# xiaguan/yalm

Measured on AMD Instinct MI355X. Metric: decode tok/s Mistral-7B fp16 @1 GPU; % of HBM bytes/token roofline, higher is better.
Workload: dtype f16; 1 GPU; mistral-7b fp16 batch-1 greedy decode, 1163 tokens, kv_len 19..1181; model=mistral-7b, global_batch=1, seq_len=1181, parallelism=single

## Files before the change

include/yalm_hip.h:

```cpp
#ifndef YALM_HIP_H
#define YALM_HIP_H

#include <stddef.h>
#include <stdint.h>

#ifdef __cplusplus
extern "C" {
#endif

#define YALM_OK 0
#define YALM_ERR_HIP 1
#define YALM_ERR_ARG 2
#define YALM_ERR_UNSUPPORTED 3

enum { YALM_F32 = 0, YALM_F16 = 1, YALM_BF16 = 2, YALM_F8E5M2 = 3 };
enum { YALM_Q4 = 16 };
enum { YALM_GELU = 0, YALM_SILU = 1 };
enum { YALM_HYDRATE_KV_CACHE = 0, YALM_OUTPUT_LOGITS = 1 };

typedef struct yalm_stream_s *yalm_stream;
typedef struct yalm_decoder_s *yalm_decoder;

typedef struct yalm_config {
	int dim, hidden_dim, head_dim, n_layers, n_heads, n_kv_heads, vocab_size, max_seq_len;
// ... 53 lines not shown
int yalm_set_x(yalm_decoder d, const float *host);
int yalm_get_logits(yalm_decoder d, float *host);
int yalm_time_kernel(yalm_decoder d, int kernel_id, int iters, float *avg_ms);
int yalm_stream_envelope(size_t bytes, int iters, float *avg_ms);
int yalm_set_gemv_config(yalm_decoder d, int kind, int threads, int unroll, int gpw);
int yalm_graph_kernels(yalm_decoder d, int mode, int *kernels, int *nodes);
const char *yalm_kernel_name(yalm_decoder d, int kernel_id);
int yalm_decoder_attn_wo(yalm_decoder d);
#define YALM_LAUNCH_EAGER 1
#define YALM_LAUNCH_SYNC 2
#define YALM_LAUNCH_SEPARATE_ATTN_WO 4
int yalm_decoder_set_launch(yalm_decoder d, int flags);
int yalm_attn_wo_plan(const yalm_config *config, int slots, int *splits, int *grid);
int yalm_attn_wo_trace(yalm_decoder d, unsigned long long *host, size_t count, int *workgroups,
                       int *attention_workgroups);

typedef struct yalm_rope_scaling {
	int type;
	float factor, low_freq_factor, high_freq_factor;
	int original_max_position;
} yalm_rope_scaling;
int yalm_decoder_set_rope_scaling(yalm_decoder d, const yalm_rope_scaling *s);
int yalm_decoder_get_inv_freq(yalm_decoder d, float *host);
int yalm_decoder_set_qkv_bias(yalm_decoder d, const float *const *bq, const float *const *bk,
                              const float *const *bv);

typedef struct yalm_moe_config {
	int n_experts, n_experts_active;
} yalm_moe_config;
int yalm_decoder_create_moe(const yalm_config *config, const yalm_moe_config *moe, const yalm_model_weights *weights,
// ... 69 lines not shown
```

yalm_amd/csrc/attention.h:

```cpp
#pragma once

#include <float.h>

#include <type_traits>

#include "device_common.h"

#define ATTN_THREADS 256
#define ATTN_SPLITS 32
#define ATTN_MAX_SPLITS 64
#define ATTN_HEAD_MAX 4
#define ATTN_WAVES (ATTN_THREADS / YALM_WAVE)

template <int D>
constexpr int attn_chunk() {
	return 64;
}

template <int D>
constexpr int attn_nk() {
	return attn_chunk<D>() / (ATTN_WAVES * (64 / (D / 8))) > 0 ? attn_chunk<D>() / (ATTN_WAVES * (64 / (D / 8))) : 1;
}

template <int D>
struct KvRows {
	static constexpr int LPK = D / 8, KPW = 64 / LPK, RSTEP = (ATTN_THREADS / 64) * KPW;
	static constexpr int NK = attn_nk<D>();
	const char *kb, *vb;
	uint32_t rowb, msl;
	uint32_t voff[NK];
	__device__ __forceinline__ KvRows(const uint16_t *kc, const uint16_t *vc, int n_kv_heads, int max_seq_len, int g) {
		const int lane = threadIdx.x & 63;
		const int tl0 = (threadIdx.x >> 6) * KPW + lane / LPK, piece = lane % LPK;
		auto uni = [](const uint16_t *p) {
			const uint64_t a = (uint64_t)p;
			const uint32_t lo = __builtin_amdgcn_readfirstlane((uint32_t)a);
// ... 105 lines not shown
	case 12: return dpp<0x15C>(v);
	case 13: return dpp<0x15D>(v);
	case 14: return dpp<0x15E>(v);
	default: return dpp<0x15F>(v);
	}
}
template <int LPK, bool MAX>
__device__ __forceinline__ float attn_wave_red(float v) {
	auto op = [](float a, float b) { return MAX ? fmaxf(a, b) : a + b; };
	v = attn_fold_row<LPK, MAX>(v);
	if constexpr (LPK <= 16)
		v = op(v, xor16(v));
	return op(v, xor32(v));
}

template <int D, int GT, int GQ, bool GRAN>
__device__ __forceinline__ bool attn_core(int g, int hq0, int Gh, int c_first, int cstride, int ns, bool final_out,
                                          int s_part, const float4_t (&qv)[(GQ * D + 255) / 256],
                                          u32x4_t (&kA)[attn_nk<D>()], u32x4_t (&vA)[attn_nk<D>()],
                                          int kv_len, const uint16_t *kc, const uint16_t *vc, int n_heads,
                                          int n_kv_heads, int max_seq_len, int nsplit, unsigned long long *part,
                                          unsigned ptag, float *out, float *att_dbg, unsigned gtag,
                                          unsigned long long *ts, bool trace_on) {
	constexpr int CHUNK = attn_chunk<D>();
	c_first = __builtin_amdgcn_readfirstlane(c_first);
	cstride = __builtin_amdgcn_readfirstlane(cstride);
	ns = __builtin_amdgcn_readfirstlane(ns);
	kv_len = __builtin_amdgcn_readfirstlane(kv_len);
	constexpr int LPK = D / 8;
	static_assert(LPK >= 2 && LPK <= 32 && (LPK & (LPK - 1)) == 0, "head_dim 16 .. 256, a power of two");
	constexpr int KPW = 64 / LPK;
	constexpr int RSTEP = ATTN_WAVES * KPW;
	constexpr int NK = CHUNK / RSTEP > 0 ? CHUNK / RSTEP : 1;
	constexpr int QL = (GQ * D + 255) / 256;
// ... 16 lines not shown
	auto stamp = [&](int k) {
		if (ts) {
			tss[k] = __builtin_amdgcn_s_memrealtime();
			tss[8 + k] = __builtin_amdgcn_s_memtime();
		}
	};
	auto flush = [&]() {
		if (ts) {
#pragma unroll
			for (int k = 2; k < 8; ++k)
				if (k != 3)
					ts[k] = tss[k], ts[8 + k] = tss[8 + k];
		}
	};
	if (trace_on) {
		asm volatile("s_waitcnt vmcnt(0)" ::: "memory");
		__syncthreads();
		stamp(2);
	}
	const int gq = G * D;
#pragma unroll
	for (int j = 0; j < QL; ++j)
		if ((j * 64 + lane) * 4 < gq)
			*(float4_t *)&qs[wave][(j * 64 + lane) * 4] = qv[j];
	float qr[GT][8];
#pragma unroll
	for (int h = 0; h < GT; ++h) {
		const float *qp = &qs[wave][(hq0 + (h < Gh ? h : 0)) * D + piece * 8];
		const float4_t a = *(const float4_t *)qp;
		const float4_t b = *(const float4_t *)(qp + 4);
		qr[h][0] = a[0], qr[h][1] = a[1], qr[h][2] = a[2], qr[h][3] = a[3];
// ... 144 lines not shown
#pragma unroll
			for (int i = 0; i < NK; ++i) {
				float vf[8];
				WF16::unpack(valid[i] ? vw[i] : u32x4_t{0u, 0u, 0u, 0u}, vf);
#pragma unroll
				for (int h = 0; h < GT; ++h)
#pragma unroll
					for (int e = 0; e < 8; ++e)
						acc[h * 8 + e] = fmaf(sv[i][h], vf[e], acc[h * 8 + e]);
			}
		}
	};

	using T_ = std::true_type;
	using F_ = std::false_type;
	if (c_first + cstride >= ns) {
		chunk(T_{}, kA, vA, c_first * CHUNK);
	} else {
		u32x4_t kB[NK], vB[NK];
		load_kv((c_first + cstride) * CHUNK, kB, vB);
		chunk(T_{}, kA, vA, c_first * CHUNK);
		for (int c = c_first + cstride;; c += 2 * cstride) {
			load_kv((c + cstride) * CHUNK, kA, vA);
			chunk(F_{}, kB, vB, c * CHUNK);
			if (c + cstride >= ns)
				break;
			load_kv((c + 2 * cstride) * CHUNK, kB, vB);
			chunk(F_{}, kA, vA, (c + cstride) * CHUNK);
			if (c + 2 * cstride >= ns)
				break;
		}
// ... 77 lines not shown
			for (int w = 1; w < ATTN_WAVES; ++w)
				M = fmaxf(M, wml[w][h][0]);
			float L = 0.0f;
#pragma unroll
			for (int w = 0; w < ATTN_WAVES; ++w)
				L = fmaf(wml[w][h][1], expf(wml[w][h][0] - M), L);
			float *a = att_dbg + (size_t)(hb + h) * max_seq_len + t;
			*a = expf(ld_sc1(a) - M) / L;
		}
	}
	flush();
	return final_out;
}

template <int D, int GT, bool GRAN>
__device__ __forceinline__ bool attn_decode_body(int g, int u, int S, int head_max, const float *q,
                                                 const uint16_t *kc, const uint16_t *vc, const StepState *step,
                                                 int n_heads, int n_kv_heads, int max_seq_len, int nsplit,
                                                 unsigned long long *part, unsigned ptag, float *out, float *att_dbg,
                                                 unsigned gtag = 0, unsigned long long *ts = nullptr,
                                                 bool trace_on = false) {
	constexpr int CHUNK = attn_chunk<D>();
	constexpr int LPK = D / 8;
	constexpr int KPW = 64 / LPK;
	constexpr int RSTEP = ATTN_WAVES * KPW;
	constexpr int NK = CHUNK / RSTEP > 0 ? CHUNK / RSTEP : 1;
	constexpr int QL = (GT * D + 255) / 256;
	const int G = n_heads / n_kv_heads;
	const int lane = threadIdx.x & 63;
	const bool hu = u < G;
	const int s = hu ? 0 : u - G + 1;
	const int gq = G * D;
	float4_t qv[QL];
#pragma unroll
	for (int j = 0; j < QL; ++j)
		qv[j] = *(const float4_t *)(q + (size_t)g * gq + min((j * 64 + lane) * 4, gq - 4));
	u32x4_t kA[NK], vA[NK];
	const KvRows<D> rows(kc, vc, n_kv_heads, max_seq_len, g);
	rows.load(0, hu, kA, vA);
	const int kv_len = step->kv_len;
	const int ns = (kv_len + CHUNK - 1) / CHUNK;
	if (ns <= head_max) {
		if (!hu)
			return false;
		return attn_core<D, 1, GT, GRAN>(g, u, 1, 0, 1, ns, true, 0, qv, kA, vA, kv_len, kc, vc, n_heads, n_kv_heads,
		                                 max_seq_len, nsplit, part, ptag, out, att_dbg, gtag, ts, trace_on);
	}
	if (s * CHUNK >= kv_len)
		return false;
	if (!hu)
		rows.load(s * CHUNK, true, kA, vA);
	if (hu)
		return attn_core<D, 1, GT, GRAN>(g, u, 1, 0, S, ns, false, 0, qv, kA, vA, kv_len, kc, vc, n_heads, n_kv_heads,
		                                 max_seq_len, nsplit, part, ptag, out, att_dbg, gtag, ts, trace_on);
	return attn_core<D, GT, GT, GRAN>(g, 0, G, s, S, ns, false, s, qv, kA, vA, kv_len, kc, vc, n_heads, n_kv_heads,
	                                  max_seq_len, nsplit, part, ptag, out, att_dbg, gtag, ts, trace_on);
}

template <int D, bool GRAN>
__device__ __forceinline__ bool attn_merge_body(int g, int hq, int S, int head_max, const StepState *step, int n_heads,
                                                int n_kv_heads, int max_seq_len, int nsplit,
                                                const unsigned long long *part, unsigned ptag, unsigned *err,
                                                float *out, float *att_dbg, unsigned gtag = 0,
                                                unsigned long long *ts = nullptr) {
	constexpr int CHUNK = attn_chunk<D>();
	constexpr int SPW = ATTN_MAX_SPLITS / ATTN_WAVES;
	constexpr int E = D >= 64 ? D / 64 : 1;
	__shared__ float mml[ATTN_WAVES][2];
	__shared__ float mo[ATTN_WAVES][D];
	const int G = n_heads / n_kv_heads;
	const int h = g * G + hq;
// ... 85 lines not shown
	for (int d = tid; d < D; d += ATTN_THREADS)
		attn_out<GRAN>(out, (size_t)h * D + d, ((mo[0][d] + mo[1][d]) + (mo[2][d] + mo[3][d])) / L, gtag);
	if (att_dbg) {
		for (int t = tid; t < kv_len; t += ATTN_THREADS) {
			float *a = att_dbg + (size_t)h * max_seq_len + t;
			*a = expf(ld_sc1(a) - M) / L;
		}
	}
	return true;
}

template <int D, int GT>
__global__ __launch_bounds__(ATTN_THREADS) void attn_decode_kernel(
    const float *__restrict__ q, const uint16_t *__restrict__ kc, const uint16_t *__restrict__ vc,
    const StepState *__restrict__ step, int n_heads, int n_kv_heads, int max_seq_len, int nsplit, int S,
    int head_max, unsigned long long *__restrict__ part, int layer, int n_layers, unsigned *__restrict__ err,
    float *__restrict__ out, float *__restrict__ att_dbg) {
	const int b = blockIdx.x, units = n_kv_heads * (S + n_heads / n_kv_heads - 1);
	const unsigned ptag = attn_part_tag(step, layer, n_layers);
	if (b < units)
		attn_decode_body<D, GT, false>(b % n_kv_heads, b / n_kv_heads, S, head_max, q, kc, vc, step, n_heads,
		                               n_kv_heads, max_seq_len, nsplit, part, ptag, out, att_dbg);
	else
		attn_merge_body<D, false>((b - units) % n_kv_heads, (b - units) / n_kv_heads, S, head_max, step, n_heads,
		                          n_kv_heads, max_seq_len, nsplit, part, ptag, err, out, att_dbg);
}
```

yalm_amd/csrc/attn_wo.h:

```cpp
#pragma once

#include "attention.h"
#include "device_common.h"
#include "tp_exchange.h"

#define AWO_RPW 16
#define AWO_TIMEOUT 200000000ull
#define AWO_REPL_STRIDE 32
#define AWO_SHORT_KV 64
#define AWO_TRACE_N 16

struct AttnWoArgs {
	int n_heads, n_kv, max_seq_len, nsplit, S;
	int head_max;
	int q_dim, dim;
	unsigned long long *part;
	int layer, n_layers;
	const unsigned long long *gran;
	const char *wo;
	float *x;
	float *out;
	int add_base;
	TpX push;
	unsigned *err;
	unsigned long long *trace;
	int delay;
};

__device__ __forceinline__ void awo_ld8_sc1(u32x4_t (&v)[8], const void *const (&a)[8]) {
// ... 97 lines not shown
	unsigned long long t_start = 0, c_start = 0;
	if (tr) {
		t_start = __builtin_amdgcn_s_memrealtime();
		c_start = (unsigned long long)__builtin_amdgcn_s_getreg((31 << 11) | 4) |
		          ((unsigned long long)__builtin_amdgcn_s_getreg((31 << 11) | 20) << 32);
	}

	const unsigned epoch = step->epoch;
	if (b < munits) {
		const unsigned ptag = epoch * (unsigned)p.n_layers + (unsigned)p.layer;
		if (tr) {
			tr[2] = tr[10] = 0;
			for (int k = 4; k < 8; ++k)
				tr[k] = tr[8 + k] = 0;
		}
		const bool wrote =
		    b < units ? attn_decode_body<D, GT, true>(b % p.n_kv, b / p.n_kv, p.S, p.head_max, q, kc, vc, step,
		                                               p.n_heads, p.n_kv, p.max_seq_len, p.nsplit, p.part, ptag,
		                                               (float *)p.gran, nullptr, epoch, tr, p.trace != nullptr)
		              : attn_merge_body<D, true>((b - units) % p.n_kv, (b - units) / p.n_kv, p.S, p.head_max, step,
		                                         p.n_heads, p.n_kv, p.max_seq_len, p.nsplit, p.part, ptag, p.err,
		                                         (float *)p.gran, nullptr, epoch, tr);
		if (tr) {
			const unsigned long long t1 = __builtin_amdgcn_s_memrealtime(), c1 = __builtin_amdgcn_s_memtime();
			tr[0] = t_start, tr[8] = c_start;
			tr[1] = wrote ? t1 : 0, tr[9] = wrote ? c1 : 0;
			tr[3] = t1, tr[11] = c1;
		}
		return;
	}

	__shared__ float rowpart[AWO_RPW][ATTN_WAVES];
// ... 83 lines not shown
```

yalm_amd/csrc/decoder.h:

```cpp
#pragma once

#include <hip/hip_runtime.h>

#include <cstdlib>
#include <string>
#include <vector>

#include "../../include/yalm_hip.h"
#include "device_common.h"
#include "tp_exchange.h"

void set_err(const std::string &s);

#define HIPCHK(expr)                                                                                                   \
	do {                                                                                                               \
		hipError_t e_ = (expr);                                                                                        \
		if (e_ != hipSuccess) {                                                                                        \
			set_err(std::string(#expr) + " failed: " + hipGetErrorString(e_) + " (" + __FILE__ + ":" +                 \
			        std::to_string(__LINE__) + ")");                                                                   \
			return YALM_ERR_HIP;                                                                                       \
		}                                                                                                              \
	} while (0)

#define ARGCHK(cond, msg)                                                                                              \
// ... 103 lines not shown
	int ipc_S = 0;
	float *ipc_own = nullptr;
	float **ipc_bufs = nullptr;
	std::vector<void *> ipc_opened;
	TpX tpx{};
	bool tpx_gate = false;
	bool tpx_collect = false;
	bool attn_wo = false, attn_wo_ok = false;
	int awo_nb = 0;
	int awo_S = 0;
	int awo_slots = 0;
	unsigned long long *awo_trace = nullptr;
	int awo_delay = 0;
	int awo_delay_short = -1;
	long long awo_kv_hint = -1;
	unsigned long long *awo_gran = nullptr;
	unsigned *awo_err = nullptr;
	int moe_E = 0, moe_K = 0;
	StepState *rstep = nullptr;
	float *rx = nullptr, *rq = nullptr, *rxb2 = nullptr, *rhb = nullptr, *rlogits = nullptr;
	float *rlogits_pinned = nullptr;
	struct SpecState *spec = nullptr;
	int *spec_ctx = nullptr;
	int *spec_stream = nullptr;
	int spec_stream_cap = 0;
	yalm_rope_scaling rope_scaling{};
	std::vector<const float *> bq, bk, bv;
	std::vector<const void *> moegate;
	int *moe_sel = nullptr;
	float *moe_wts = nullptr;
// ... 5 lines not shown
```

yalm_amd/csrc/yalm_hip.hip:

```cpp
#include "../../include/yalm_hip.h"

#include <hip/hip_runtime.h>
#include <rccl/rccl.h>

#include <algorithm>
#include <cmath>
#include <cstddef>
#include <cstdio>
#include <cstdlib>
#include <cstring>
#include <string>
#include <vector>

#include "attention.h"
#include "attn_wo.h"
#include "decoder.h"
#include "device_common.h"
#include "gemv.h"
#include "gemv_rows.h"
#include "misc_kernels.h"
#include "moe.h"
#include "sampler.h"
#include "spec.h"

// ... 415 lines not shown
	ARGCHK(n_experts >= 1 && n_experts <= MOE_MAX_EXPERTS && n_active >= 1 && n_active <= n_experts,
	       "mixture of experts: need 1 <= n_experts_active <= n_experts <= 64");
	return YALM_OK;
}

static bool attn_supported(int head_dim, int G) {
	return (head_dim == 16 || head_dim == 32 || head_dim == 64 || head_dim == 128 || head_dim == 256) && G >= 1 &&
	       G <= 8;
}

static int attn_head_max(int S, int nchunks) {
	static const int h = ab_env("YALM_ATTN_HEADMAX") ? atoi(ab_env("YALM_ATTN_HEADMAX")) : ATTN_HEAD_MAX;
	return S <= 1 ? nchunks : std::max(1, h);
}

template <int D>
static void launch_attn_D(int G, const float *q, const uint16_t *kc, const uint16_t *vc, const StepState *step,
                          int n_heads, int n_kv, int max_seq_len, int nsplit, unsigned long long *part, int layer,
                          int n_layers, unsigned *err, float *att, float *out, hipStream_t st) {
	static const int splits = ab_env("YALM_ATTN_SPLITS") ? std::max(1, std::min(ATTN_MAX_SPLITS, atoi(ab_env("YALM_ATTN_SPLITS")))) : ATTN_SPLITS;
	const int nchunks = (max_seq_len + attn_chunk<D>() - 1) / attn_chunk<D>();
	const int S = std::min(nchunks, splits);
	const int grid = n_kv * (S + G - 1) + n_heads;
	const int hmax = attn_head_max(S, nchunks);
#define YALM_ATTN(GT)                                                                                                  \
	attn_decode_kernel<D, GT><<<grid, ATTN_THREADS, 0, st>>>(q, kc, vc, step, n_heads, n_kv, max_seq_len, nsplit, S, \
	                                                         hmax, part, layer, n_layers, err, out, att)
	if (G <= 1)
		YALM_ATTN(1);
	else if (G <= 2)
		YALM_ATTN(2);
	else if (G <= 4)
		YALM_ATTN(4);
	else
		YALM_ATTN(8);
#undef YALM_ATTN
}

static int attn_nsplit(int max_seq_len) {
	return (max_seq_len + attn_chunk<128>() - 1) / attn_chunk<128>();
}

static int launch_attn(int head_dim, int n_heads, int n_kv, const float *q, const uint16_t *kc, const uint16_t *vc,
                       const StepState *step, int max_seq_len, unsigned long long *part, int layer, int n_layers,
                       unsigned *err, float *att,
                       float *out, hipStream_t st) {
	const int G = n_heads / n_kv;
	const int nsplit = attn_nsplit(max_seq_len);
	switch (head_dim) {
	case 16:
		launch_attn_D<16>(G, q, kc, vc, step, n_heads, n_kv, max_seq_len, nsplit, part, layer, n_layers, err, att,
		                   out, st);
		break;
	case 32:
		launch_attn_D<32>(G, q, kc, vc, step, n_heads, n_kv, max_seq_len, nsplit, part, layer, n_layers, err, att,
		                   out, st);
		break;
	case 64:
		launch_attn_D<64>(G, q, kc, vc, step, n_heads, n_kv, max_seq_len, nsplit, part, layer, n_layers, err, att,
		                   out, st);
		break;
	case 128:
		launch_attn_D<128>(G, q, kc, vc, step, n_heads, n_kv, max_seq_len, nsplit, part, layer, n_layers, err, att,
		                   out, st);
		break;
	case 256:
		launch_attn_D<256>(G, q, kc, vc, step, n_heads, n_kv, max_seq_len, nsplit, part, layer, n_layers, err, att,
		                   out, st);
		break;
	default:
		set_err("unsupported head_dim");
		return YALM_ERR_UNSUPPORTED;
	}
	HIPCHK(hipGetLastError());
	return YALM_OK;
}

template <class WT, int GT, int KB>
static const void *attn_wo_fn() {
	return (const void *)attn_wo_kernel<WT, GT, KB>;
}
template <class WT, int KB>
static const void *attn_wo_fn_g(int G) {
// ... 120 lines not shown
	else if (G <= 4)
		launch_attn_wo_k<WT, 4, KB>(d, w, p);
	else
		launch_attn_wo_k<WT, 8, KB>(d, w, p);
}
template <class WT>
static int launch_attn_wo(yalm_decoder_s *d, const yalm_block_weights &w, int layer, int ex) {
	const yalm_config &c = d->c;
	AttnWoArgs p;
	p.n_heads = c.n_heads;
	p.n_kv = c.n_kv_heads;
	p.max_seq_len = c.max_seq_len;
	p.nsplit = attn_nsplit(c.max_seq_len);
	p.S = d->awo_S;
	p.head_max = attn_head_max(d->awo_S, (c.max_seq_len + attn_chunk<128>() - 1) / attn_chunk<128>());
	p.q_dim = c.n_heads * c.head_dim;
	p.dim = c.dim;
	p.part = d->part;
	p.layer = layer;
	p.n_layers = c.n_layers;
	p.gran = d->awo_gran + (size_t)layer * p.q_dim;
	p.wo = (const char *)w.wo;
	p.x = d->x;
	p.out = d->comm ? d->xs : d->x;
	p.add_base = d->tp_rank == 0;
	p.push = d->ipc ? tpx_ex(d, ex) : TpX{};
	p.err = d->awo_err;
	p.trace = d->awo_trace;
	p.delay = d->awo_delay_short >= 0 && d->awo_kv_hint >= 0 && d->awo_kv_hint <= AWO_SHORT_KV ? d->awo_delay_short
	                                                                                         : d->awo_delay;
// ... 145 lines not shown
	const yalm_block_weights &w = d->b[l];
	hipStream_t st = d->stream;
	const int q_dim = c.n_heads * c.head_dim;
	const TpX none{};
	if (!d->bq.empty()) {
		TRY((launch_gemv_d<WT, PQKVB<WT>, true>(d, make_pqkvb<WT>(d, l), d->x, w.rms_att, c.norm_eps, GK_QKV, none)));
	} else {
		const PQKV<WT> p = make_pqkv<WT>(d, w);
		TRY((launch_gemv_d<WT, PQKV<WT>, true>(d, p, d->x, w.rms_att, c.norm_eps, GK_QKV,
		                                         d->ipc && x_exchanged ? tpx_consume(d, ex0 - 1, c.dim) : none)));
	}
	if (d->attn_wo && wt_fused_wo<WT>()) {
		TRY(launch_attn_wo<WT>(d, w, l, ex0));
	} else {
		TRY(launch_attn(c.head_dim, c.n_heads, c.n_kv_heads, d->q, w.key_cache, w.value_cache, d->step, c.max_seq_len,
		                d->part, l, c.n_layers, d->awo_err, nullptr, d->xb2, st));
		TRY(enqueue_residual_gemv<WT>(d, w.wo, q_dim, d->xb2, GK_WO, ex0));
	}
	if constexpr (!WT::Q4) {
		if (d->moe_E > 0) {
			const MoeArgs a = moe_layer_args(d, l);
			TRY((launch_moe_router<WT, true>(a, d->x, w.rms_ffn, c.norm_eps, st)));
			TRY((launch_moe_glu<WT, true>(a, d->x, w.rms_ffn, c.norm_eps, d->gemv[GK_GLU], st)));
			return launch_moe_w2<WT>(a, d->x, d->gemv[GK_W2], st);
		}
	}
	if (c.act == YALM_SILU) {
		PGlu<WT, 1> p;
		p.w1 = (const char *)w.w1;
		p.w3 = (const char *)w.w3;
		p.n = c.dim;
// ... 108 lines not shown
		HIPCHK(hipGetLastError());
		if (ncclAllGather(d->amax, d->amax_all, 2, ncclFloat, (ncclComm_t)d->comm, d->stream) != ncclSuccess) {
			set_err("ncclAllGather (argmax) failed");
			return YALM_ERR_HIP;
		}
		argmax_pick_kernel<<<1, 1, 0, d->stream>>>(d->amax_all, d->tp_size, d->step, d->tokens, d->tokens_cap);
		HIPCHK(hipGetLastError());
	}
	return YALM_OK;
}

static int ensure_graph(yalm_decoder_s *d, int which) {
	if (d->exec[which] || d->eager)
		return YALM_OK;
	HIPCHK(hipStreamBeginCapture(d->stream, hipStreamCaptureModeRelaxed));
	int r = enqueue_forward(d, which);
	hipGraph_t g = nullptr;
	hipError_t e = hipStreamEndCapture(d->stream, &g);
	if (r != YALM_OK)
		return r;
	HIPCHK(e);
	d->graph[which] = g;
	HIPCHK(hipGraphInstantiate(&d->exec[which], g, nullptr, nullptr, 0));
	return YALM_OK;
}

static void drop_graphs(yalm_decoder_s *d) {
	for (int i = 0; i < N_GRAPHS; ++i) {
		if (d->exec[i])
			(void)hipGraphExecDestroy(d->exec[i]);
		if (d->graph[i])
// ... 647 lines not shown
				p.q_stride = q_dim;
				TRY((launch_rows<WT, RQKVB<WT>, true>(p, d->rx, c.dim, w.rms_att, c.norm_eps, T, st)));
			} else {
				RQKV<WT> p;
				p.base = make_pqkv<WT>(d, w);
				p.base.step = d->rstep;
				p.base.q_out = d->rq;
				p.n = c.dim;
				p.n_groups = p.base.n_groups;
				p.q_stride = q_dim;
				TRY((launch_rows<WT, RQKV<WT>, true>(p, d->rx, c.dim, w.rms_att, c.norm_eps, T, st)));
			}
			for (int t = 0; t < T; ++t)
				TRY(launch_attn(c.head_dim, c.n_heads, c.n_kv_heads, d->rq + (size_t)t * q_dim, w.key_cache,
				                w.value_cache, d->rstep + t, c.max_seq_len, d->part, l, c.n_layers, d->awo_err, nullptr,
				                d->rxb2 + (size_t)t * q_dim, st));
			{
				RResidual<WT> p;
				p.W = (const char *)w.wo;
				p.n = q_dim;
				p.n_rows = c.dim;
				p.n_groups = (c.dim + 1) / 2;
				p.out = d->rx;
				p.ostride = c.dim;
				TRY((launch_rows<WT, RResidual<WT>, false>(p, d->rxb2, q_dim, nullptr, 0.f, T, st)));
			}
			if (c.act == YALM_SILU)
				TRY((launch_rows_glu<WT, 1>(d, w, T)));
			else
				TRY((launch_rows_glu<WT, 0>(d, w, T)));
			{
// ... 269 lines not shown
			p.out = d->x;
			p.n_groups = c.dim;
			return launch_gemv_d<WT, PResidual<WT, 1>, false>(d, p, kernel_id == 2 ? d->xb2 : d->hb, nullptr, 0.f,
			                                                  kernel_id == 2 ? GK_WO : GK_W2);
		}
		PGlu<WT, 1> p;
		p.w1 = (const char *)w.w1;
		p.w3 = (const char *)w.w3;
		p.n = c.dim;
		p.out = d->hb;
		p.n_groups = c.hidden_dim;
		return launch_gemv_d<WT, PGlu<WT, 1>, true>(d, p, d->x, w.rms_ffn, c.norm_eps, GK_GLU);
	}
	case 1:
		return launch_attn(c.head_dim, c.n_heads, c.n_kv_heads, d->q, w.key_cache, w.value_cache, d->step,
		                   c.max_seq_len, d->part, l, c.n_layers, d->awo_err, nullptr, d->xb2, d->stream);
	case 5:
		return enqueue_logits_t<WT>(d, -1, -1);
	case 6:
		return enqueue_exchange(d);
	case 8:
		if constexpr (wt_fused_wo<WT>())
			return launch_attn_wo<WT>(d, w, l, 0);
		break;
	case 10:
		sample_kernel<<<1, SMP_THREADS, 0, d->stream>>>(d->logits, c.vocab_size, d->smp_params, d->smp_u, 1,
		                                                d->smp_step, nullptr, 0, nullptr, nullptr);
		HIPCHK(hipGetLastError());
		return YALM_OK;
	}
	set_err("bad kernel_id");
// ... 28 lines not shown
extern "C" int yalm_decoder_set_launch(yalm_decoder d, int flags) {
	ARGCHK(d, "null decoder");
	ARGCHK(!(flags & ~(YALM_LAUNCH_EAGER | YALM_LAUNCH_SYNC | YALM_LAUNCH_SEPARATE_ATTN_WO)), "unknown launch flag");
	HIPCHK(hipStreamSynchronize(d->stream));
	drop_graphs(d);
	d->eager = flags & YALM_LAUNCH_EAGER;
	d->graph_sync = flags & YALM_LAUNCH_SYNC;
	d->attn_wo = d->attn_wo_ok && !(flags & YALM_LAUNCH_SEPARATE_ATTN_WO);
	return YALM_OK;
}

extern "C" int yalm_decoder_attn_wo(yalm_decoder d) {
	return d && d->attn_wo ? 1 : 0;
}

extern "C" int yalm_attn_wo_trace(yalm_decoder d, unsigned long long *host, size_t count, int *workgroups,
                                  int *attention_workgroups) {
	ARGCHK(d && host, "null argument");
	ARGCHK(d->attn_wo && d->awo_trace, "no attn_wo trace (create the decoder with YALM_ATTN_WO_TRACE=1)");
	HIPCHK(hipStreamSynchronize(d->stream));
	const size_t total = (size_t)AWO_TRACE_N * d->awo_nb;
	HIPCHK(hipMemcpy(host, d->awo_trace, sizeof(unsigned long long) * std::min(count, total), hipMemcpyDeviceToHost));
	if (workgroups)
		*workgroups = d->awo_nb;
	if (attention_workgroups)
		*attention_workgroups = d->c.n_kv_heads * (d->awo_S + d->c.n_heads / d->c.n_kv_heads - 1) + d->c.n_heads;
	return YALM_OK;
}

static int time_loop(yalm_decoder_s *d, int kernel_id, int iters, bool bump, bool kernel, float *ms_out) {
// ... 17 lines not shown
	*ms_out = ms / iters;
	return r;
}

extern "C" int yalm_time_kernel(yalm_decoder d, int kernel_id, int iters, float *avg_ms) {
	ARGCHK(d && avg_ms && iters > 0 && kernel_id >= 0 && kernel_id <= 10 && kernel_id != 7,
	       "bad argument (kernel ids 0-6, 8, 9, 10)");
	ARGCHK(kernel_id != 10 || (d->tp_size == 1 && !d->comm && !d->ipc && d->c.vocab_size <= SMP_MAX_N),
	       "kernel 10 (device sampling) needs a one-GPU decoder and a vocabulary of at most 131072");
	ARGCHK(kernel_id != 9 || d->moe_E > 0, "kernel 9 (expert router) needs a mixture-of-experts decoder");
	ARGCHK(kernel_id != 6 || d->comm || d->ipc, "kernel 6 (tensor-parallel exchange) needs a tensor-parallel decoder");
	ARGCHK(kernel_id != 8 || d->attn_wo, "kernel 8 (fused attention + Wo) needs yalm_decoder_attn_wo");
	const bool bump = kernel_id == 1 || kernel_id == 8 || (kernel_id == 6 && d->ipc);
	if (bump)
		epoch_bump_kernel<<<1, 1, 0, d->stream>>>(d->step, 1);
	TRY(DISPATCH_WT(d->c.weight_dtype, enqueue_one_t, d, kernel_id, 0));
	float ms = 0.f;
	TRY(time_loop(d, kernel_id, iters, bump, true, &ms));
	if (bump) {
		float mb = 0.f;
		TRY(time_loop(d, kernel_id, iters, true, false, &mb));
		ms = std::max(0.f, ms - mb);
	}
	TRY(awo_check(d));
	*avg_ms = ms;
	return YALM_OK;
}

extern "C" int yalm_set_gemv_config(yalm_decoder d, int kind, int threads, int unroll, int gpw) {
	ARGCHK(d && kind >= 0 && kind < GK_N, "bad decoder/kind");
// ... 191 lines not shown
	}
	const size_t kvn = (size_t)max_seq_len * n_kv_heads * head_dim;
	const int nsplit = attn_nsplit(max_seq_len);
	DevBuf dk, dv, dq, dout, datt, dpart, dstep, derr;
	TRY(up(dk, kb, kvn * 2));
	TRY(up(dv, vb, kvn * 2));
	TRY(up(dq, q, sizeof(float) * n_heads * head_dim));
	TRY(up(dout, nullptr, sizeof(float) * n_heads * head_dim));
	TRY(up(datt, att, sizeof(float) * (size_t)n_heads * max_seq_len));
	TRY(up(dpart, nullptr, sizeof(unsigned long long) * (size_t)n_heads * nsplit * (head_dim + 2)));
	TRY(up(dstep, nullptr, sizeof(StepState)));
	TRY(up(derr, nullptr, sizeof(unsigned)));
	set_step_full_kernel<<<1, 1>>>((StepState *)dstep.p, kv_len - 1, 0, kv_len - 1, kv_len);
	TRY(launch_attn(head_dim, n_heads, n_kv_heads, (const float *)dq.p, (const uint16_t *)dk.p,
	                (const uint16_t *)dv.p, (const StepState *)dstep.p, max_seq_len, (unsigned long long *)dpart.p, 0, 1,
	                (unsigned *)derr.p, att ? (float *)datt.p : nullptr, (float *)dout.p, nullptr));
	HIPCHK(hipDeviceSynchronize());
	HIPCHK(hipMemcpy(xout, dout.p, sizeof(float) * n_heads * head_dim, hipMemcpyDeviceToHost));
	if (att)
		HIPCHK(hipMemcpy(att, datt.p, sizeof(float) * (size_t)n_heads * max_seq_len, hipMemcpyDeviceToHost));
	unsigned e = 0;
	HIPCHK(hipMemcpy(&e, derr.p, sizeof(e), hipMemcpyDeviceToHost));
	if (e) {
		set_err("yalm_mha: the split-KV merger gave up waiting for a chunk");
		return YALM_ERR_HIP;
	}
	return YALM_OK;
}

extern "C" int yalm_argmax(const float *logits, int n, int n_shards, int *out) {
	ARGCHK(logits && out && n > 0 && n_shards >= 1 && n_shards <= 64 && n % n_shards == 0, "yalm_argmax: bad argument");
// ... 142 lines not shown
```

yalm_amd/runtime.py:

```python

from __future__ import annotations

import ctypes
import os

import numpy as np

from . import models as M

HERE = os.path.dirname(os.path.abspath(__file__))
LIB_PATH = os.environ.get("YALM_LIB") or os.path.join(HERE, "libyalm_hip.so")

if not os.path.exists(LIB_PATH):
    raise ImportError(
        f"{LIB_PATH} is missing: build it with `make -C {os.path.dirname(HERE)}` "
        "(or __graft_entry__.build()). There is no CPU fallback."
    )

lib = ctypes.CDLL(LIB_PATH)

c_void_p = ctypes.c_void_p
c_int = ctypes.c_int
c_float = ctypes.c_float
c_size_t = ctypes.c_size_t
# ... 104 lines not shown
_sig("yalm_enqueue_greedy", c_int, [c_void_p, c_int])
_sig("yalm_generate_sampled", c_int, [c_void_p, c_int, c_int, c_int, ctypes.POINTER(Sampling), c_void_p, c_void_p])
_sig("yalm_sample", c_int, [c_void_p, c_int, ctypes.POINTER(Sampling), c_void_p, c_int, c_void_p, c_void_p, c_void_p])
_sig("yalm_device_step", c_int, [c_void_p, ctypes.POINTER(c_int), ctypes.POINTER(c_int)])
_sig("yalm_device_tokens", c_int, [c_void_p, c_void_p, c_int, ctypes.POINTER(c_int)])
_sig("yalm_block", c_int, [c_void_p, c_int, c_int, c_int, c_int, c_int])
_sig("yalm_get_x", c_int, [c_void_p, c_void_p])
_sig("yalm_set_x", c_int, [c_void_p, c_void_p])
_sig("yalm_get_logits", c_int, [c_void_p, c_void_p])
_sig("yalm_time_kernel", c_int, [c_void_p, c_int, c_int, ctypes.POINTER(c_float)])
_sig("yalm_kernel_name", ctypes.c_char_p, [c_void_p, c_int])
_sig("yalm_set_gemv_config", c_int, [c_void_p, c_int, c_int, c_int, c_int])
_sig("yalm_stream_envelope", c_int, [ctypes.c_size_t, c_int, ctypes.POINTER(c_float)])
_sig("yalm_decoder_attn_wo", c_int, [c_void_p])
_sig("yalm_attn_wo_trace", c_int, [c_void_p, c_void_p, ctypes.c_size_t, ctypes.POINTER(c_int), ctypes.POINTER(c_int)])
_sig("yalm_matmul", c_int, [c_void_p, c_void_p, c_void_p, c_int, c_int, c_int])
_sig("yalm_mha", c_int, [c_void_p, c_void_p, c_void_p, c_void_p, c_void_p, c_int, c_int, c_int, c_int, c_int])
_sig("yalm_argmax", c_int, [c_void_p, c_int, c_int, ctypes.POINTER(c_int)])
_sig("yalm_ffn", c_int, [c_void_p, c_void_p, c_void_p, c_void_p, c_void_p, c_int, c_int, c_int, c_int])
_sig("yalm_prefill", c_int, [c_void_p, c_void_p, c_int, c_int, c_void_p])
_sig("yalm_tp_unique_id", c_int, [c_void_p])
_sig("yalm_decoder_create_tp", c_int, [c_void_p, c_void_p, c_int, c_int, c_void_p, c_void_p, c_void_p])
_sig("yalm_tp_ipc_alloc", c_int, [c_void_p, c_int, c_void_p, ctypes.POINTER(c_void_p), c_void_p])
_sig("yalm_stream_create_cu_part", c_int, [c_int, c_int, ctypes.POINTER(c_void_p)])
_sig("yalm_decoder_set_launch", c_int, [c_void_p, c_int])
_sig("yalm_decoder_create_tp_ipc", c_int, [c_void_p, c_void_p, c_int, c_int, c_void_p, c_void_p, c_void_p, c_void_p])
_sig("yalm_copy_2d", c_int, [c_void_p, ctypes.c_size_t, c_void_p, ctypes.c_size_t, ctypes.c_size_t, ctypes.c_size_t])
_sig("yalm_prefill_time", c_int, [c_void_p, c_int, c_int, ctypes.POINTER(c_float)])
_sig("yalm_prefill_info", c_int, [c_void_p, ctypes.POINTER(c_int), ctypes.POINTER(c_int)])
_sig("yalm_set_prefill_precision", c_int, [c_void_p, c_int])
# ... 15 lines not shown
    "yalm_unregister_host", "yalm_free", "yalm_stream_create", "yalm_stream_destroy", "yalm_stream_sync",
    "yalm_synth", "yalm_decoder_create", "yalm_decoder_destroy", "yalm_forward", "yalm_generate_greedy",
    "yalm_enqueue_greedy", "yalm_device_step", "yalm_device_tokens", "yalm_block", "yalm_get_x", "yalm_set_x", "yalm_get_logits",
    "yalm_time_kernel", "yalm_kernel_name", "yalm_set_gemv_config", "yalm_matmul", "yalm_mha", "yalm_ffn",
    "yalm_prefill", "yalm_prefill_time", "yalm_gemm_f16", "yalm_attn_prefill", "yalm_tp_unique_id",
    "yalm_decoder_create_tp", "yalm_copy_2d", "yalm_tp_ipc_alloc", "yalm_decoder_create_tp_ipc",
    "yalm_decoder_attn_wo", "yalm_attn_wo_trace", "yalm_stream_envelope",
    "yalm_argmax", "yalm_set_prefill_forms", "yalm_attn_wo_plan", "yalm_graph_kernels",
    "yalm_stream_create_cu_part", "yalm_decoder_set_launch", "yalm_prefill_info", "yalm_set_prefill_precision",
    "yalm_decoder_create_moe", "yalm_moe_routing", "yalm_moe_ffn",
    "yalm_prefill_routing", "yalm_moe_gemm_f16", "yalm_moe_ffn_rows",
    "yalm_generate_sampled", "yalm_sample",
    "yalm_row_bytes", "yalm_synth_q4",
    "yalm_forward_rows", "yalm_generate_speculative", "yalm_spec_draft",
    "yalm_decoder_set_rope_scaling", "yalm_decoder_get_inv_freq", "yalm_decoder_set_qkv_bias",
]
PREFILL_FAST, PREFILL_SPLIT = 0, 1

HYDRATE_KV_CACHE, OUTPUT_LOGITS = 0, 1
LAUNCH_EAGER, LAUNCH_SYNC, LAUNCH_SEPARATE_ATTN_WO = 1, 2, 4
TP_HANDLE_BYTES = 128


class YalmError(RuntimeError):
    pass


def check(rc: int) -> None:
    if rc != 0:
        raise YalmError(f"yalm error {rc}: {lib.yalm_last_error().decode()}")
# ... 473 lines not shown
        check(lib.yalm_moe_routing(self.h, _ptr(experts), _ptr(weights)))
        return experts, weights

    def time_kernel(self, kernel_id: int, iters: int) -> float:
        ms = c_float()
        check(lib.yalm_time_kernel(self.h, kernel_id, iters, ctypes.byref(ms)))
        return ms.value

    def set_gemv_config(self, kind: int, threads: int = 0, unroll: int = 0, gpw: int = 0) -> None:
        check(lib.yalm_set_gemv_config(self.h, kind, threads, unroll, gpw))

    @property
    def attn_wo(self) -> bool:
        return bool(lib.yalm_decoder_attn_wo(self.h))

    def attn_wo_trace(self):
        buf = np.zeros(16 * 8192, np.uint64)
        nb, na = c_int(), c_int()
        check(lib.yalm_attn_wo_trace(self.h, buf.ctypes.data, buf.size, ctypes.byref(nb), ctypes.byref(na)))
        return buf[: 16 * nb.value].reshape(nb.value, 16), na.value

    def graph_kernels(self, mode: int = 2) -> int:
        k, n = c_int(), c_int()
        check(lib.yalm_graph_kernels(self.h, mode, ctypes.byref(k), ctypes.byref(n)))
        return k.value

    def kernel_name(self, kernel_id: int) -> str:
        return lib.yalm_kernel_name(self.h, kernel_id).decode()

    def close(self):
# ... 13 lines not shown
```

Baseline: 391.0 tok/s.

## Prefetch KV chunks through a multi-buffer ring in single-unit decode attention

Adds a register ring of up to four KV chunk buffers for head_dim up to 128, so a head's attention unit issues loads for several chunks before computing, then alternates two buffers as a lookahead. An optional host-supplied kv-length hint lets the ring loads start before the step's kv_len is read from device memory, with a new API to skew or disable the hint; the hint is cleared during graph capture and set only for kernel timing. The non-hinted single-unit path with two or more chunks also uses the ring, so it runs in the normal graph decode. It trades extra VGPRs, which may lower occupancy, for deeper memory-level parallelism, and adds a full vmcnt wait at the start of the fused attn_wo path.

After: 391.3 tok/s (median of 2 runs). About the same (+0.1%).

```diff
diff --git a/include/yalm_hip.h b/include/yalm_hip.h
--- a/include/yalm_hip.h
+++ b/include/yalm_hip.h
@@ -91,6 +91,7 @@
 int yalm_attn_wo_plan(const yalm_config *config, int slots, int *splits, int *grid);
 int yalm_attn_wo_trace(yalm_decoder d, unsigned long long *host, size_t count, int *workgroups,
                        int *attention_workgroups);
+int yalm_decoder_set_kv_hint_skew(yalm_decoder d, int mode, int keys);
 
 typedef struct yalm_rope_scaling {
 	int type;
diff --git a/yalm_amd/csrc/attention.h b/yalm_amd/csrc/attention.h
--- a/yalm_amd/csrc/attention.h
+++ b/yalm_amd/csrc/attention.h
@@ -20,6 +20,16 @@
 template <int D>
 constexpr int attn_nk() {
 	return attn_chunk<D>() / (ATTN_WAVES * (64 / (D / 8))) > 0 ? attn_chunk<D>() / (ATTN_WAVES * (64 / (D / 8))) : 1;
+}
+
+#define ATTN_HEAD_RING 4
+template <int D>
+constexpr int attn_ring() {
+	return D <= 128 ? ATTN_HEAD_RING : 1;
+}
+template <int D>
+constexpr int attn_ring_bufs() {
+	return attn_ring<D>() > 1 ? attn_ring<D>() - 1 : 1;
 }
 
 template <int D>
@@ -155,10 +165,12 @@
 	return op(v, xor32(v));
 }
 
-template <int D, int GT, int GQ, bool GRAN>
+template <int D, int GT, int GQ, bool GRAN, bool RINGED>
 __device__ __forceinline__ bool attn_core(int g, int hq0, int Gh, int c_first, int cstride, int ns, bool final_out,
                                           int s_part, const float4_t (&qv)[(GQ * D + 255) / 256],
                                           u32x4_t (&kA)[attn_nk<D>()], u32x4_t (&vA)[attn_nk<D>()],
+                                          u32x4_t (&kR)[attn_ring_bufs<D>()][attn_nk<D>()],
+                                          u32x4_t (&vR)[attn_ring_bufs<D>()][attn_nk<D>()], int nring,
                                           int kv_len, const uint16_t *kc, const uint16_t *vc, int n_heads,
                                           int n_kv_heads, int max_seq_len, int nsplit, unsigned long long *part,
                                           unsigned ptag, float *out, float *att_dbg, unsigned gtag,
@@ -205,7 +217,10 @@
 		}
 	};
 	if (trace_on) {
-		asm volatile("s_waitcnt vmcnt(0)" ::: "memory");
+		if constexpr (RINGED)
+			asm volatile("s_waitcnt vmcnt(%0)" ::"n"(2 * (attn_ring<D>() - 1) * attn_nk<D>()) : "memory");
+		else
+			asm volatile("s_waitcnt vmcnt(0)" ::: "memory");
 		__syncthreads();
 		stamp(2);
 	}
@@ -380,7 +395,30 @@
 
 	using T_ = std::true_type;
 	using F_ = std::false_type;
-	if (c_first + cstride >= ns) {
+	if constexpr (RINGED) {
+		constexpr int R = attn_ring<D>();
+		const int nr = min(ns, __builtin_amdgcn_readfirstlane(nring));
+		chunk(T_{}, kA, vA, 0);
+#pragma unroll
+		for (int r = 1; r < R; ++r)
+			if (r < nr)
+				chunk(F_{}, kR[r - 1], vR[r - 1], r * CHUNK);
+		if (nr < ns) {
+			static_assert(R >= 3, "the lookahead alternates between the ring's first two buffers");
+			constexpr int B = 1;
+			load_kv(nr * CHUNK, kR[B], vR[B]);
+			for (int c = nr;; c += 2) {
+				load_kv((c + 1) * CHUNK, kR[0], vR[0]);
+				chunk(F_{}, kR[B], vR[B], c * CHUNK);
+				if (c + 1 >= ns)
+					break;
+				load_kv((c + 2) * CHUNK, kR[B], vR[B]);
+				chunk(F_{}, kR[0], vR[0], (c + 1) * CHUNK);
+				if (c + 2 >= ns)
+					break;
+			}
+		}
+	} else if (c_first + cstride >= ns) {
 		chunk(T_{}, kA, vA, c_first * CHUNK);
 	} else {
 		u32x4_t kB[NK], vB[NK];
@@ -488,7 +526,7 @@
 }
 
 template <int D, int GT, bool GRAN>
-__device__ __forceinline__ bool attn_decode_body(int g, int u, int S, int head_max, const float *q,
+__device__ __forceinline__ bool attn_decode_body(int g, int u, int S, int head_max, int kv_hint, const float *q,
                                                  const uint16_t *kc, const uint16_t *vc, const StepState *step,
                                                  int n_heads, int n_kv_heads, int max_seq_len, int nsplit,
                                                  unsigned long long *part, unsigned ptag, float *out, float *att_dbg,
@@ -512,23 +550,59 @@
 	u32x4_t kA[NK], vA[NK];
 	const KvRows<D> rows(kc, vc, n_kv_heads, max_seq_len, g);
 	rows.load(0, hu, kA, vA);
-	const int kv_len = step->kv_len;
+	constexpr int RING = attn_ring<D>(), RB = RING > 1 ? RING - 1 : 1;
+	u32x4_t kR[RB][NK], vR[RB][NK];
+	auto ring_load = [&](int keys) {
+#pragma unroll
+		for (int r = 1; r < RING; ++r)
+			rows.load(r * CHUNK, r * CHUNK < keys, kR[r - 1], vR[r - 1]);
+	};
+	const int hkeys = __builtin_amdgcn_readfirstlane(min(kv_hint, max_seq_len));
+	const int hns = (hkeys + CHUNK - 1) / CHUNK;
+	const bool hinted = RING > 1 && hu && hns >= 2 && hns <= head_max;
+	int kv_len = step->kv_len;
+	if (hinted) {
+		ring_load(hkeys);
+		asm volatile("" : "+s"(kv_len)::"memory");
+		const int ns = (kv_len + CHUNK - 1) / CHUNK;
+		if (ns <= head_max)
+			return attn_core<D, 1, GT, GRAN, (RING > 1)>(g, u, 1, 0, 1, ns, true, 0, qv, kA, vA, kR, vR, min(hns, RING),
+			                                       kv_len, kc, vc, n_heads, n_kv_heads, max_seq_len, nsplit, part, ptag,
+			                                       out, att_dbg, gtag, ts, trace_on);
+	} else {
+		asm volatile("" : "+s"(kv_len)::"memory");
+		const int ns = (kv_len + CHUNK - 1) / CHUNK;
+		if (ns <= head_max) {
+			if (!hu)
+				return false;
+			if constexpr (RING > 1) {
+				if (ns == 1)
+					return attn_core<D, 1, GT, GRAN, false>(g, u, 1, 0, 1, 1, true, 0, qv, kA, vA, kR, vR, 1, kv_len, kc,
+					                                        vc, n_heads, n_kv_heads, max_seq_len, nsplit, part, ptag,
+					                                        out, att_dbg, gtag, ts, trace_on);
+				ring_load(kv_len);
+				return attn_core<D, 1, GT, GRAN, true>(g, u, 1, 0, 1, ns, true, 0, qv, kA, vA, kR, vR, RING, kv_len, kc,
+				                                       vc, n_heads, n_kv_heads, max_seq_len, nsplit, part, ptag, out,
+				                                       att_dbg, gtag, ts, trace_on);
+			} else {
+				return attn_core<D, 1, GT, GRAN, false>(g, u, 1, 0, 1, ns, true, 0, qv, kA, vA, kR, vR, 1, kv_len, kc, vc,
+				                                        n_heads, n_kv_heads, max_seq_len, nsplit, part, ptag, out,
+				                                        att_dbg, gtag, ts, trace_on);
+			}
+		}
+	}
 	const int ns = (kv_len + CHUNK - 1) / CHUNK;
-	if (ns <= head_max) {
-		if (!hu)
-			return false;
-		return attn_core<D, 1, GT, GRAN>(g, u, 1, 0, 1, ns, true, 0, qv, kA, vA, kv_len, kc, vc, n_heads, n_kv_heads,
-		                                 max_seq_len, nsplit, part, ptag, out, att_dbg, gtag, ts, trace_on);
-	}
 	if (s * CHUNK >= kv_len)
 		return false;
 	if (!hu)
 		rows.load(s * CHUNK, true, kA, vA);
 	if (hu)
-		return attn_core<D, 1, GT, GRAN>(g, u, 1, 0, S, ns, false, 0, qv, kA, vA, kv_len, kc, vc, n_heads, n_kv_heads,
-		                                 max_seq_len, nsplit, part, ptag, out, att_dbg, gtag, ts, trace_on);
-	return attn_core<D, GT, GT, GRAN>(g, 0, G, s, S, ns, false, s, qv, kA, vA, kv_len, kc, vc, n_heads, n_kv_heads,
-	                                  max_seq_len, nsplit, part, ptag, out, att_dbg, gtag, ts, trace_on);
+		return attn_core<D, 1, GT, GRAN, false>(g, u, 1, 0, S, ns, false, 0, qv, kA, vA, kR, vR, 1, kv_len, kc, vc,
+		                                        n_heads, n_kv_heads, max_seq_len, nsplit, part, ptag, out, att_dbg,
+		                                        gtag, ts, trace_on);
+	return attn_core<D, GT, GT, GRAN, false>(g, 0, G, s, S, ns, false, s, qv, kA, vA, kR, vR, 1, kv_len, kc, vc, n_heads,
+	                                         n_kv_heads, max_seq_len, nsplit, part, ptag, out, att_dbg, gtag, ts,
+	                                         trace_on);
 }
 
 template <int D, bool GRAN>
@@ -644,12 +718,12 @@
 __global__ __launch_bounds__(ATTN_THREADS) void attn_decode_kernel(
     const float *__restrict__ q, const uint16_t *__restrict__ kc, const uint16_t *__restrict__ vc,
     const StepState *__restrict__ step, int n_heads, int n_kv_heads, int max_seq_len, int nsplit, int S,
-    int head_max, unsigned long long *__restrict__ part, int layer, int n_layers, unsigned *__restrict__ err,
-    float *__restrict__ out, float *__restrict__ att_dbg) {
+    int head_max, int kv_hint, unsigned long long *__restrict__ part, int layer, int n_layers,
+    unsigned *__restrict__ err, float *__restrict__ out, float *__restrict__ att_dbg) {
 	const int b = blockIdx.x, units = n_kv_heads * (S + n_heads / n_kv_heads - 1);
 	const unsigned ptag = attn_part_tag(step, layer, n_layers);
 	if (b < units)
-		attn_decode_body<D, GT, false>(b % n_kv_heads, b / n_kv_heads, S, head_max, q, kc, vc, step, n_heads,
+		attn_decode_body<D, GT, false>(b % n_kv_heads, b / n_kv_heads, S, head_max, kv_hint, q, kc, vc, step, n_heads,
 		                               n_kv_heads, max_seq_len, nsplit, part, ptag, out, att_dbg);
 	else
 		attn_merge_body<D, false>((b - units) % n_kv_heads, (b - units) / n_kv_heads, S, head_max, step, n_heads,
diff --git a/yalm_amd/csrc/attn_wo.h b/yalm_amd/csrc/attn_wo.h
--- a/yalm_amd/csrc/attn_wo.h
+++ b/yalm_amd/csrc/attn_wo.h
@@ -13,6 +13,7 @@
 struct AttnWoArgs {
 	int n_heads, n_kv, max_seq_len, nsplit, S;
 	int head_max;
+	int kv_hint;
 	int q_dim, dim;
 	unsigned long long *part;
 	int layer, n_layers;
@@ -140,8 +141,9 @@
 			for (int k = 4; k < 8; ++k)
 				tr[k] = tr[8 + k] = 0;
 		}
+		__builtin_amdgcn_s_waitcnt(0x0F70);
 		const bool wrote =
-		    b < units ? attn_decode_body<D, GT, true>(b % p.n_kv, b / p.n_kv, p.S, p.head_max, q, kc, vc, step,
+		    b < units ? attn_decode_body<D, GT, true>(b % p.n_kv, b / p.n_kv, p.S, p.head_max, p.kv_hint, q, kc, vc, step,
 		                                               p.n_heads, p.n_kv, p.max_seq_len, p.nsplit, p.part, ptag,
 		                                               (float *)p.gran, nullptr, epoch, tr, p.trace != nullptr)
 		              : attn_merge_body<D, true>((b - units) % p.n_kv, (b - units) / p.n_kv, p.S, p.head_max, step,
diff --git a/yalm_amd/csrc/decoder.h b/yalm_amd/csrc/decoder.h
--- a/yalm_amd/csrc/decoder.h
+++ b/yalm_amd/csrc/decoder.h
@@ -141,6 +141,7 @@
 	int awo_delay = 0;
 	int awo_delay_short = -1;
 	long long awo_kv_hint = -1;
+	int kv_hint_mode = 0, kv_hint_keys = 0;
 	unsigned long long *awo_gran = nullptr;
 	unsigned *awo_err = nullptr;
 	int moe_E = 0, moe_K = 0;
diff --git a/yalm_amd/csrc/yalm_hip.hip b/yalm_amd/csrc/yalm_hip.hip
--- a/yalm_amd/csrc/yalm_hip.hip
+++ b/yalm_amd/csrc/yalm_hip.hip
@@ -453,10 +453,17 @@
 	return S <= 1 ? nchunks : std::max(1, h);
 }
 
+static int attn_kv_hint(const yalm_decoder_s *d) {
+	if (d->awo_kv_hint < 0 || d->kv_hint_mode == 2)
+		return 0;
+	long long h = d->awo_kv_hint + (d->kv_hint_mode == 1 ? d->kv_hint_keys : 0);
+	return (int)std::max<long long>(1, std::min<long long>(h, d->c.max_seq_len));
+}
+
 template <int D>
 static void launch_attn_D(int G, const float *q, const uint16_t *kc, const uint16_t *vc, const StepState *step,
                           int n_heads, int n_kv, int max_seq_len, int nsplit, unsigned long long *part, int layer,
-                          int n_layers, unsigned *err, float *att, float *out, hipStream_t st) {
+                          int n_layers, unsigned *err, float *att, float *out, int kv_hint, hipStream_t st) {
 	static const int splits = ab_env("YALM_ATTN_SPLITS") ? std::max(1, std::min(ATTN_MAX_SPLITS, atoi(ab_env("YALM_ATTN_SPLITS")))) : ATTN_SPLITS;
 	const int nchunks = (max_seq_len + attn_chunk<D>() - 1) / attn_chunk<D>();
 	const int S = std::min(nchunks, splits);
@@ -464,7 +471,7 @@
 	const int hmax = attn_head_max(S, nchunks);
 #define YALM_ATTN(GT)                                                                                                  \
 	attn_decode_kernel<D, GT><<<grid, ATTN_THREADS, 0, st>>>(q, kc, vc, step, n_heads, n_kv, max_seq_len, nsplit, S, \
-	                                                         hmax, part, layer, n_layers, err, out, att)
+	                                                         hmax, kv_hint, part, layer, n_layers, err, out, att)
 	if (G <= 1)
 		YALM_ATTN(1);
 	else if (G <= 2)
@@ -483,29 +490,29 @@
 static int launch_attn(int head_dim, int n_heads, int n_kv, const float *q, const uint16_t *kc, const uint16_t *vc,
                        const StepState *step, int max_seq_len, unsigned long long *part, int layer, int n_layers,
                        unsigned *err, float *att,
-                       float *out, hipStream_t st) {
+                       float *out, int kv_hint, hipStream_t st) {
 	const int G = n_heads / n_kv;
 	const int nsplit = attn_nsplit(max_seq_len);
 	switch (head_dim) {
 	case 16:
 		launch_attn_D<16>(G, q, kc, vc, step, n_heads, n_kv, max_seq_len, nsplit, part, layer, n_layers, err, att,
-		                   out, st);
+		                   out, kv_hint, st);
 		break;
 	case 32:
 		launch_attn_D<32>(G, q, kc, vc, step, n_heads, n_kv, max_seq_len, nsplit, part, layer, n_layers, err, att,
-		                   out, st);
+		                   out, kv_hint, st);
 		break;
 	case 64:
 		launch_attn_D<64>(G, q, kc, vc, step, n_heads, n_kv, max_seq_len, nsplit, part, layer, n_layers, err, att,
-		                   out, st);
+		                   out, kv_hint, st);
 		break;
 	case 128:
 		launch_attn_D<128>(G, q, kc, vc, step, n_heads, n_kv, max_seq_len, nsplit, part, layer, n_layers, err, att,
-		                   out, st);
+		                   out, kv_hint, st);
 		break;
 	case 256:
 		launch_attn_D<256>(G, q, kc, vc, step, n_heads, n_kv, max_seq_len, nsplit, part, layer, n_layers, err, att,
-		                   out, st);
+		                   out, kv_hint, st);
 		break;
 	default:
 		set_err("unsupported head_dim");
@@ -656,6 +663,7 @@
 	p.nsplit = attn_nsplit(c.max_seq_len);
 	p.S = d->awo_S;
 	p.head_max = attn_head_max(d->awo_S, (c.max_seq_len + attn_chunk<128>() - 1) / attn_chunk<128>());
+	p.kv_hint = attn_kv_hint(d);
 	p.q_dim = c.n_heads * c.head_dim;
 	p.dim = c.dim;
 	p.part = d->part;
@@ -831,7 +839,7 @@
 		TRY(launch_attn_wo<WT>(d, w, l, ex0));
 	} else {
 		TRY(launch_attn(c.head_dim, c.n_heads, c.n_kv_heads, d->q, w.key_cache, w.value_cache, d->step, c.max_seq_len,
-		                d->part, l, c.n_layers, d->awo_err, nullptr, d->xb2, st));
+		                d->part, l, c.n_layers, d->awo_err, nullptr, d->xb2, attn_kv_hint(d), st));
 		TRY(enqueue_residual_gemv<WT>(d, w.wo, q_dim, d->xb2, GK_WO, ex0));
 	}
 	if constexpr (!WT::Q4) {
@@ -970,7 +978,10 @@
 	if (d->exec[which] || d->eager)
 		return YALM_OK;
 	HIPCHK(hipStreamBeginCapture(d->stream, hipStreamCaptureModeRelaxed));
+	const long long hint = d->awo_kv_hint;
+	d->awo_kv_hint = -1;
 	int r = enqueue_forward(d, which);
+	d->awo_kv_hint = hint;
 	hipGraph_t g = nullptr;
 	hipError_t e = hipStreamEndCapture(d->stream, &g);
 	if (r != YALM_OK)
@@ -1648,7 +1659,7 @@
 			for (int t = 0; t < T; ++t)
 				TRY(launch_attn(c.head_dim, c.n_heads, c.n_kv_heads, d->rq + (size_t)t * q_dim, w.key_cache,
 				                w.value_cache, d->rstep + t, c.max_seq_len, d->part, l, c.n_layers, d->awo_err, nullptr,
-				                d->rxb2 + (size_t)t * q_dim, st));
+				                d->rxb2 + (size_t)t * q_dim, 0, st));
 			{
 				RResidual<WT> p;
 				p.W = (const char *)w.wo;
@@ -1948,7 +1959,7 @@
 	}
 	case 1:
 		return launch_attn(c.head_dim, c.n_heads, c.n_kv_heads, d->q, w.key_cache, w.value_cache, d->step,
-		                   c.max_seq_len, d->part, l, c.n_layers, d->awo_err, nullptr, d->xb2, d->stream);
+		                   c.max_seq_len, d->part, l, c.n_layers, d->awo_err, nullptr, d->xb2, attn_kv_hint(d), d->stream);
 	case 5:
 		return enqueue_logits_t<WT>(d, -1, -1);
 	case 6:
@@ -2007,6 +2018,13 @@
 	return d && d->attn_wo ? 1 : 0;
 }
 
+extern "C" int yalm_decoder_set_kv_hint_skew(yalm_decoder d, int mode, int keys) {
+	ARGCHK(d && mode >= 0 && mode <= 2, "yalm_decoder_set_kv_hint_skew: mode 0 (exact), 1 (hint + keys) or 2 (unknown)");
+	d->kv_hint_mode = mode;
+	d->kv_hint_keys = mode == 1 ? keys : 0;
+	return YALM_OK;
+}
+
 extern "C" int yalm_attn_wo_trace(yalm_decoder d, unsigned long long *host, size_t count, int *workgroups,
                                   int *attention_workgroups) {
 	ARGCHK(d && host, "null argument");
@@ -2054,6 +2072,12 @@
 	const bool bump = kernel_id == 1 || kernel_id == 8 || (kernel_id == 6 && d->ipc);
 	if (bump)
 		epoch_bump_kernel<<<1, 1, 0, d->stream>>>(d->step, 1);
+	struct HintScope {
+		yalm_decoder_s *d;
+		~HintScope() { d->awo_kv_hint = -1; }
+	} hint_scope{d};
+	if ((kernel_id == 1 || kernel_id == 8) && d->host_pos >= 0)
+		d->awo_kv_hint = std::min<long long>(d->host_pos + 1, d->c.max_seq_len);
 	TRY(DISPATCH_WT(d->c.weight_dtype, enqueue_one_t, d, kernel_id, 0));
 	float ms = 0.f;
 	TRY(time_loop(d, kernel_id, iters, bump, true, &ms));
@@ -2275,7 +2299,7 @@
 	set_step_full_kernel<<<1, 1>>>((StepState *)dstep.p, kv_len - 1, 0, kv_len - 1, kv_len);
 	TRY(launch_attn(head_dim, n_heads, n_kv_heads, (const float *)dq.p, (const uint16_t *)dk.p,
 	                (const uint16_t *)dv.p, (const StepState *)dstep.p, max_seq_len, (unsigned long long *)dpart.p, 0, 1,
-	                (unsigned *)derr.p, att ? (float *)datt.p : nullptr, (float *)dout.p, nullptr));
+	                (unsigned *)derr.p, att ? (float *)datt.p : nullptr, (float *)dout.p, 0, nullptr));
 	HIPCHK(hipDeviceSynchronize());
 	HIPCHK(hipMemcpy(xout, dout.p, sizeof(float) * n_heads * head_dim, hipMemcpyDeviceToHost));
 	if (att)
diff --git a/yalm_amd/runtime.py b/yalm_amd/runtime.py
--- a/yalm_amd/runtime.py
+++ b/yalm_amd/runtime.py
@@ -142,6 +142,7 @@
 _sig("yalm_stream_envelope", c_int, [ctypes.c_size_t, c_int, ctypes.POINTER(c_float)])
 _sig("yalm_decoder_attn_wo", c_int, [c_void_p])
 _sig("yalm_attn_wo_trace", c_int, [c_void_p, c_void_p, ctypes.c_size_t, ctypes.POINTER(c_int), ctypes.POINTER(c_int)])
+_sig("yalm_decoder_set_kv_hint_skew", c_int, [c_void_p, c_int, c_int])
 _sig("yalm_matmul", c_int, [c_void_p, c_void_p, c_void_p, c_int, c_int, c_int])
 _sig("yalm_mha", c_int, [c_void_p, c_void_p, c_void_p, c_void_p, c_void_p, c_int, c_int, c_int, c_int, c_int])
 _sig("yalm_argmax", c_int, [c_void_p, c_int, c_int, ctypes.POINTER(c_int)])
@@ -187,6 +188,7 @@
     "yalm_row_bytes", "yalm_synth_q4",
     "yalm_forward_rows", "yalm_generate_speculative", "yalm_spec_draft",
     "yalm_decoder_set_rope_scaling", "yalm_decoder_get_inv_freq", "yalm_decoder_set_qkv_bias",
+    "yalm_decoder_set_kv_hint_skew",
 ]
 PREFILL_FAST, PREFILL_SPLIT = 0, 1
 
@@ -690,6 +692,11 @@
     def attn_wo(self) -> bool:
         return bool(lib.yalm_decoder_attn_wo(self.h))
 
+    KV_HINT_EXACT, KV_HINT_SKEW, KV_HINT_UNKNOWN = 0, 1, 2
+
+    def set_kv_hint_skew(self, mode: int = 0, keys: int = 0) -> None:
+        check(lib.yalm_decoder_set_kv_hint_skew(self.h, mode, keys))
+
     def attn_wo_trace(self):
         buf = np.zeros(16 * 8192, np.uint64)
         nb, na = c_int(), c_int()
```
